# kmaninis/OSVOS-PyTorch

Hardware: NVIDIA H100
Metric: frames/sec at 480x854 fwd-only, batch 1 per GPU (OSVOS.forward -> 5 logit maps) (higher is better)
Workload: dtype bf16x3 (split-bf16 operands, fp32 accumulate)

## Files before the change

osvos_pytorch_b200/csrc/conv_stage1_fused.cu:

```cuda
#include <stdlib.h>
#include <string.h>

#include "conv_common.cuh"

namespace osvos {

constexpr int kS1Pitch = 10;
constexpr int kS1HaloRows = kTileH + 2;
constexpr int kS1HaloPx = kS1HaloRows * kS1Pitch;
constexpr int kS1APlane = (kS1HaloPx * 128 + 1023) / 1024 * 1024;
constexpr int kS1AStage = 2 * kS1APlane;
constexpr int kS1AStages = 2;
constexpr int kS1BPlane = 64 * 128;
constexpr int kS1BStage = 2 * kS1BPlane;
constexpr int kS1BStages = 5;
constexpr int kS1W1Bytes = (64 * 27 + 64) * 4;
constexpr int kS1Builders = 96;
constexpr int kS1Smem = kS1AStages * kS1AStage + kS1BStages * kS1BStage + kS1W1Bytes + 1024 + 512;
static_assert(kS1Smem <= 227 * 1024, "stage-1 kernel exceeds the per-CTA shared memory");
static_assert(kS1Smem + 4096 < (1 << 18), "descriptor start-address field would overflow");

struct Stage1Params {
  const float* x;
  const float* w1;
  const float* b1;
};

__global__ void __launch_bounds__(kConvThreads, 1)
conv_stage1_fused_kernel(const __grid_constant__ CUtensorMap map_w_hi, const __grid_constant__ CUtensorMap map_w_lo,
                         const Stage1Params s1, const ConvParams p) {
  extern __shared__ uint8_t smem_raw[];
  uint8_t* smem = reinterpret_cast<uint8_t*>((reinterpret_cast<uintptr_t>(smem_raw) + 1023) & ~uintptr_t(1023));
  uint8_t* smem_a = smem;
  uint8_t* smem_b = smem_a + kS1AStages * kS1AStage;
  float* w1s = reinterpret_cast<float*>(smem_b + kS1BStages * kS1BStage);
  uint64_t* bars = reinterpret_cast<uint64_t*>(reinterpret_cast<uint8_t*>(w1s) + kS1W1Bytes);
  uint64_t* a_full = bars;
  uint64_t* a_empty = bars + 2;
  uint64_t* b_full = bars + 4;
  uint64_t* b_empty = bars + 4 + kS1BStages;

  const int warp = threadIdx.x >> 5;
  const int lane = threadIdx.x & 31;

  if (threadIdx.x == 0) {
    tma_prefetch_desc(&map_w_hi);
    tma_prefetch_desc(&map_w_lo);
    for (int i = 0; i < 2; ++i) {
      mbar_init(&a_full[i], kS1Builders);
      mbar_init(&a_empty[i], 2);
    }
    for (int i = 0; i < kS1BStages; ++i) {
      mbar_init(&b_full[i], 1);
      mbar_init(&b_empty[i], 2);
    }
    fence_barrier_init();
  }
  pdl_wait();
  pdl_launch_dependents();
  for (int i = threadIdx.x; i < 64 * 27 + 64; i += kConvThreads)
    w1s[i] = i < 64 * 27 ? __ldg(s1.w1 + i) : (s1.b1 ? __ldg(s1.b1 + i - 64 * 27) : 0.f);
  __syncthreads();

  if (warp == 0) {
    if (elect_one()) {
      int b_stage = 0;
      uint32_t b_phase = 0;
      for (int tile = blockIdx.x; tile < p.total_tiles; tile += gridDim.x) {
#pragma unroll
        for (int tap = 0; tap < 9; ++tap) {
          mbar_wait(&b_empty[b_stage], b_phase ^ 1);
          uint8_t* st = smem_b + b_stage * kS1BStage;
          mbar_arrive_expect_tx(&b_full[b_stage], kS1BStage);
          tma_load_3d(&map_w_hi, &b_full[b_stage], st, 0, 0, tap);
          tma_load_3d(&map_w_lo, &b_full[b_stage], st + kS1BPlane, 0, 0, tap);
          if (++b_stage == kS1BStages) {
            b_stage = 0;
            b_phase ^= 1;
          }
        }
      }
    }
    __syncwarp();
  } else if (warp < 4) {
    const int t = threadIdx.x - 32;
    const size_t plane_sz = static_cast<size_t>(p.h) * p.w;
    int a_stage = 0;
    uint32_t a_phase = 0;
    for (int tile = blockIdx.x; tile < p.total_tiles; tile += gridDim.x) {
      int nb, tx, ty, img;
      decode_tile(p, tile, nb, tx, ty, img);
      mbar_wait(&a_empty[a_stage], a_phase ^ 1);
      uint8_t* st = smem_a + a_stage * kS1AStage;
      for (int pix = t; pix < kS1HaloPx; pix += kS1Builders) {
        const int hy = pix / kS1Pitch, hx = pix - hy * kS1Pitch;
        const int y = ty * kTileH - 1 + hy, xx = tx * kTileW - 1 + hx;
        const bool inside = y >= 0 && y < p.h && xx >= 0 && xx < p.w;
        float v[27];
#pragma unroll
        for (int ci = 0; ci < 3; ++ci) {
          const float* pl = s1.x + (static_cast<size_t>(img) * 3 + ci) * plane_sz;
#pragma unroll
          for (int r = 0; r < 3; ++r) {
            const int iy = y + r - 1;
#pragma unroll
            for (int s = 0; s < 3; ++s) {
              const int ix = xx + s - 1;
              v[ci * 9 + r * 3 + s] =
                  (inside && iy >= 0 && iy < p.h && ix >= 0 && ix < p.w) ? __ldg(pl + static_cast<size_t>(iy) * p.w + ix) : 0.f;
            }
          }
        }
#pragma unroll 1
        for (int chunk = 0; chunk < 8; ++chunk) {
          float f[8];
#pragma unroll
          for (int e = 0; e < 8; ++e) {
            const int co = chunk * 8 + e;
            float acc = w1s[64 * 27 + co];
#pragma unroll
            for (int k = 0; k < 27; ++k) acc = fmaf(w1s[co * 27 + k], v[k], acc);
            f[e] = inside ? fmaxf(acc, 0.f) : 0.f;
          }
          uint32_t hi[4], lo[4];
#pragma unroll
          for (int e = 0; e < 4; ++e) split_pack2(f[2 * e], f[2 * e + 1], hi[e], lo[e]);
          const uint32_t off = sw128_offset(pix, chunk);
          *reinterpret_cast<uint4*>(st + off) = make_uint4(hi[0], hi[1], hi[2], hi[3]);
          *reinterpret_cast<uint4*>(st + kS1APlane + off) = make_uint4(lo[0], lo[1], lo[2], lo[3]);
        }
      }
      fence_proxy_async_smem();
      mbar_arrive(&a_full[a_stage]);
      if (++a_stage == kS1AStages) {
        a_stage = 0;
        a_phase ^= 1;
      }
    }
  } else {
    const int wg = (warp - 4) >> 2, wl = warp & 3;
    const bool leader = (threadIdx.x & 127) == 0;
    constexpr uint64_t kDescA = desc_template(16, kS1Pitch * 128, kDescSW128);
    constexpr uint64_t kDescB = desc_template(16, 1024, kDescSW128);
    const uint32_t smem_a_u32 = smem_u32(smem_a) + wg * 8 * kS1Pitch * 128, smem_b_u32 = smem_u32(smem_b);
    float acc[64];
    int a_stage = 0, b_stage = 0;
    uint32_t a_phase = 0, b_phase = 0;
    StageRelease pending;
    for (int tile = blockIdx.x; tile < p.total_tiles; tile += gridDim.x) {
#pragma unroll
      for (int i = 0; i < 64; ++i) acc[i] = 0.f;
      mbar_wait(&a_full[a_stage], a_phase);
      const uint64_t da0 = kDescA | static_cast<uint64_t>((smem_a_u32 + a_stage * kS1AStage) >> 4);
#pragma unroll
      for (int tap = 0; tap < 9; ++tap) {
        const uint32_t tap_off = static_cast<uint32_t>(((tap / 3) * kS1Pitch + (tap % 3)) * (128 >> 4));
        mbar_wait(&b_full[b_stage], b_phase);
        const uint64_t db_hi = kDescB | static_cast<uint64_t>((smem_b_u32 + b_stage * kS1BStage) >> 4);
        const uint64_t da_hi = da0 + tap_off;
        const uint64_t da_lo = da_hi + (kS1APlane >> 4);
        wgmma_fence();
#pragma unroll
        for (int k = 0; k < kBlockK / 16; ++k) {
          wgmma_bf16<128>(acc, da_hi + 2 * k, db_hi + 2 * k, 1);
          wgmma_bf16<64>(acc, da_lo + 2 * k, db_hi + 2 * k, 1);
        }
        wgmma_commit();
        wgmma_wait<1>();
        pending.release(leader);
        pending.bar_b = &b_empty[b_stage];
        if (tap == 8) pending.bar_a = &a_empty[a_stage];
        if (++b_stage == kS1BStages) {
          b_stage = 0;
          b_phase ^= 1;
        }
      }
      if (++a_stage == kS1AStages) {
        a_stage = 0;
        a_phase ^= 1;
      }
      wgmma_wait<0>();
      wgmma_fence_operands(acc);
      pending.release(leader);
      conv_epilogue<64, true, true>(p, acc, tile, wg, wl, lane);
    }
  }
}

}

using namespace osvos;

extern "C" int osvos_stage1_fused(const osvos_stage1_args* a, osvos_stream_t stream_) {
  OSVOS_CHECK_ARG(a != nullptr && a->x != nullptr && a->w1 != nullptr && a->w2_packed != nullptr);
  OSVOS_CHECK_ARG(a->n > 0 && a->h > 0 && a->w > 0 && a->h <= 65535 && a->n <= 65535);
  OSVOS_CHECK_ARG((a->y_hi != nullptr && a->y_lo != nullptr) || (a->pool_hi != nullptr && a->pool_lo != nullptr));
  OSVOS_CHECK_ARG((a->y_hi == nullptr) == (a->y_lo == nullptr) && (a->pool_hi == nullptr) == (a->pool_lo == nullptr));
  {
    const uintptr_t any = reinterpret_cast<uintptr_t>(a->y_hi) | reinterpret_cast<uintptr_t>(a->y_lo) |
                          reinterpret_cast<uintptr_t>(a->pool_hi) | reinterpret_cast<uintptr_t>(a->pool_lo);
    OSVOS_CHECK_ARG((any & 3) == 0);
    OSVOS_CHECK_ARG(((reinterpret_cast<uintptr_t>(a->b1) | reinterpret_cast<uintptr_t>(a->b2) |
                      reinterpret_cast<uintptr_t>(a->w2_packed)) & 15) == 0);
  }
  cudaStream_t stream = static_cast<cudaStream_t>(stream_);
  osvos_conv3x3_args c;
  memset(&c, 0, sizeof(c));
  c.w_packed = a->w2_packed;
  c.bias = a->b2;
  c.y_hi = a->y_hi;
  c.y_lo = a->y_lo;
  c.pool_hi = a->pool_hi;
  c.pool_lo = a->pool_lo;
  c.n = a->n, c.h = a->h, c.w = a->w, c.cin = 64, c.cout = 64;
  c.flags = OSVOS_FLAG_RELU;
  ConvParams p;
  fill_conv_params(p, &c, 64);
  CUtensorMap mw_hi, mw_lo;
  int rc = encode_weight_maps(&mw_hi, &mw_lo, &c, 64);
  if (rc) return rc;
  Stage1Params s1;
  s1.x = a->x;
  s1.w1 = a->w1;
  s1.b1 = a->b1;
  const int sms = device_sm_count();
  const int grid = p.total_tiles < sms ? p.total_tiles : sms;
  auto kern = conv_stage1_fused_kernel;
  static uint64_t attr_done = 0;
  OSVOS_CHECK_CUDA(ensure_dynamic_smem(kern, kS1Smem, &attr_done));
  OSVOS_CHECK_CUDA(launch_pdl(kern, dim3(grid), dim3(kConvThreads), kS1Smem, stream, mw_hi, mw_lo, s1, p));
  return OSVOS_OK;
}
```

osvos_pytorch_b200/csrc/ptx.cuh:

```cuda
#pragma once
#include <cuda.h>
#include <cuda_runtime.h>
#include <stdint.h>

#include "wgmma.cuh"

namespace osvos {

#ifndef OSVOS_SPIN_LIMIT
#define OSVOS_SPIN_LIMIT (1u << 26)
#endif

__device__ __forceinline__ uint32_t smem_u32(const void* p) {
  return static_cast<uint32_t>(__cvta_generic_to_shared(p));
}

__device__ __forceinline__ bool elect_one() {
  uint32_t pred = 0;
  asm volatile(
      "{\n\t.reg .pred P;\n\t"
      "elect.sync _|P, 0xffffffff;\n\t"
      "selp.u32 %0, 1, 0, P;\n\t}\n"
      : "=r"(pred));
  return pred != 0;
}

__device__ __forceinline__ void pdl_wait() { asm volatile("griddepcontrol.wait;" ::: "memory"); }
__device__ __forceinline__ void pdl_launch_dependents() { asm volatile("griddepcontrol.launch_dependents;" ::: "memory"); }

__device__ __forceinline__ void mbar_init(uint64_t* bar, uint32_t count) {
  asm volatile("mbarrier.init.shared::cta.b64 [%0], %1;" ::"r"(smem_u32(bar)), "r"(count) : "memory");
}
__device__ __forceinline__ void fence_barrier_init() {
  asm volatile("fence.mbarrier_init.release.cluster;" ::: "memory");
}
__device__ __forceinline__ void fence_proxy_async_smem() {
  asm volatile("fence.proxy.async.shared::cta;" ::: "memory");
}
__device__ __forceinline__ void mbar_arrive_expect_tx(uint64_t* bar, uint32_t bytes) {
  asm volatile("mbarrier.arrive.expect_tx.shared::cta.b64 _, [%0], %1;" ::"r"(smem_u32(bar)), "r"(bytes)
               : "memory");
}
__device__ __forceinline__ void mbar_arrive(uint64_t* bar) {
  asm volatile("mbarrier.arrive.shared::cta.b64 _, [%0];" ::"r"(smem_u32(bar)) : "memory");
}
__device__ __forceinline__ bool mbar_try_wait(uint64_t* bar, uint32_t parity) {
  uint32_t ok;
  asm volatile(
      "{\n\t.reg .pred P;\n\t"
      "mbarrier.try_wait.parity.shared::cta.b64 P, [%1], %2;\n\t"
      "selp.u32 %0, 1, 0, P;\n\t}\n"
      : "=r"(ok)
      : "r"(smem_u32(bar)), "r"(parity)
      : "memory");
  return ok != 0;
}

__device__ __forceinline__ void mbar_wait(uint64_t* bar, uint32_t parity) {
  uint32_t spins = 0;
  while (!mbar_try_wait(bar, parity)) {
    if (++spins > OSVOS_SPIN_LIMIT) __trap();
  }
}

__device__ __forceinline__ void cp_async_8_zfill(void* dst, const void* src, uint32_t src_bytes) {
  asm volatile("cp.async.ca.shared.global [%0], [%1], 8, %2;" ::"r"(smem_u32(dst)), "l"(src), "r"(src_bytes) : "memory");
}
__device__ __forceinline__ void cp_async_mbar_arrive_noinc(uint64_t* bar) {
  asm volatile("cp.async.mbarrier.arrive.noinc.shared::cta.b64 [%0];" ::"r"(smem_u32(bar)) : "memory");
}

__device__ __forceinline__ void tma_prefetch_desc(const CUtensorMap* m) {
  asm volatile("prefetch.tensormap [%0];" ::"l"(reinterpret_cast<uint64_t>(m)) : "memory");
}
__device__ __forceinline__ void tma_load_4d(const CUtensorMap* m, uint64_t* bar, void* dst, int c0, int c1, int c2,
                                            int c3) {
  asm volatile(
      "cp.async.bulk.tensor.4d.shared::cluster.global.mbarrier::complete_tx::bytes"
      " [%0], [%1, {%3, %4, %5, %6}], [%2];"
      ::"r"(smem_u32(dst)), "l"(reinterpret_cast<uint64_t>(m)), "r"(smem_u32(bar)), "r"(c0), "r"(c1), "r"(c2),
      "r"(c3)
      : "memory");
}
__device__ __forceinline__ void tma_load_2d(const CUtensorMap* m, uint64_t* bar, void* dst, int c0, int c1) {
  asm volatile(
      "cp.async.bulk.tensor.2d.shared::cluster.global.mbarrier::complete_tx::bytes"
      " [%0], [%1, {%3, %4}], [%2];"
      ::"r"(smem_u32(dst)), "l"(reinterpret_cast<uint64_t>(m)), "r"(smem_u32(bar)), "r"(c0), "r"(c1)
      : "memory");
}
__device__ __forceinline__ void tma_load_3d(const CUtensorMap* m, uint64_t* bar, void* dst, int c0, int c1, int c2) {
  asm volatile(
      "cp.async.bulk.tensor.3d.shared::cluster.global.mbarrier::complete_tx::bytes"
      " [%0], [%1, {%3, %4, %5}], [%2];"
      ::"r"(smem_u32(dst)), "l"(reinterpret_cast<uint64_t>(m)), "r"(smem_u32(bar)), "r"(c0), "r"(c1), "r"(c2)
      : "memory");
}
__device__ __forceinline__ void st_shared_u32(uint32_t addr, uint32_t v) {
  asm volatile("st.shared.u32 [%0], %1;" ::"r"(addr), "r"(v) : "memory");
}
__device__ __forceinline__ void tma_store_4d(const CUtensorMap* m, const void* src, int c0, int c1, int c2, int c3) {
  asm volatile(
      "cp.async.bulk.tensor.4d.global.shared::cta.bulk_group [%0, {%2, %3, %4, %5}], [%1];"
      ::"l"(reinterpret_cast<uint64_t>(m)), "r"(smem_u32(src)), "r"(c0), "r"(c1), "r"(c2), "r"(c3)
      : "memory");
}
__device__ __forceinline__ void bulk_commit_group() { asm volatile("cp.async.bulk.commit_group;" ::: "memory"); }
template <int N>
__device__ __forceinline__ void bulk_wait_group_read() { asm volatile("cp.async.bulk.wait_group.read %0;" ::"n"(N) : "memory"); }
template <int N>
__device__ __forceinline__ void bulk_wait_group() { asm volatile("cp.async.bulk.wait_group %0;" ::"n"(N) : "memory"); }

constexpr uint64_t kDescSW128 = 1ull << 62;
__host__ __device__ constexpr uint64_t desc_template(uint32_t lbo_bytes, uint32_t sbo_bytes, uint64_t layout) {
  return (static_cast<uint64_t>((lbo_bytes >> 4) & 0x3FFF) << 16) | (static_cast<uint64_t>((sbo_bytes >> 4) & 0x3FFF) << 32) |
         layout;
}
__device__ __forceinline__ uint64_t make_smem_desc(const void* p, uint32_t lbo_bytes, uint32_t sbo_bytes, uint64_t layout) {
  return desc_template(lbo_bytes, sbo_bytes, layout) | static_cast<uint64_t>((smem_u32(p) >> 4) & 0x3FFF);
}

__device__ __forceinline__ void named_bar_sync(int id, int nthreads) {
  asm volatile("bar.sync %0, %1;" ::"r"(id), "r"(nthreads) : "memory");
}
__device__ __forceinline__ void named_bar_arrive(int id, int nthreads) {
  asm volatile("bar.arrive %0, %1;" ::"r"(id), "r"(nthreads) : "memory");
}

template <int N>
__device__ __forceinline__ void setmaxnreg_dec() { asm volatile("setmaxnreg.dec.sync.aligned.u32 %0;" ::"n"(N)); }
template <int N>
__device__ __forceinline__ void setmaxnreg_inc() { asm volatile("setmaxnreg.inc.sync.aligned.u32 %0;" ::"n"(N)); }

struct StageRelease {
  uint64_t* bar_b = nullptr;
  uint64_t* bar_a = nullptr;
  __device__ __forceinline__ void release(bool leader) {
    if (leader) {
      if (bar_b) mbar_arrive(bar_b);
      if (bar_a) mbar_arrive(bar_a);
    }
    bar_b = bar_a = nullptr;
  }
};

}
```

osvos_pytorch_b200/csrc/wgmma.cuh:

```cuda
#pragma once
#include <stdint.h>

namespace osvos {

template <int N, int TA = 0, int TB = 0>
__device__ __forceinline__ void wgmma_bf16(float* d, uint64_t desc_a, uint64_t desc_b, uint32_t scale_d);

#define OSVOS_WGMMA_16(TA, TB)                                                                               \
  template <>                                                                                                  \
  __device__ __forceinline__ void wgmma_bf16<16, TA, TB>(float* d, uint64_t desc_a, uint64_t desc_b, uint32_t scale_d) { \
    asm volatile(                                                                                              \
        "{\n.reg .pred p;\nsetp.ne.b32 p, %10, 0;\n"                                                              \
        "wgmma.mma_async.sync.aligned.m64n16k16.f32.bf16.bf16 {%0, %1, %2, %3, %4, %5, %6, %7}, %8, %9, p, 1, 1, " #TA ", " #TB ";\n}\n" \
        : "+f"(d[0]), "+f"(d[1]), "+f"(d[2]), "+f"(d[3]), "+f"(d[4]), "+f"(d[5]), "+f"(d[6]), "+f"(d[7])                                                                                               \
        : "l"(desc_a), "l"(desc_b), "r"(scale_d) : "memory");                                                           \
  }
OSVOS_WGMMA_16(0, 0)
OSVOS_WGMMA_16(1, 1)
#undef OSVOS_WGMMA_16

#define OSVOS_WGMMA_32(TA, TB)                                                                               \
  template <>                                                                                                  \
  __device__ __forceinline__ void wgmma_bf16<32, TA, TB>(float* d, uint64_t desc_a, uint64_t desc_b, uint32_t scale_d) { \
    asm volatile(                                                                                              \
        "{\n.reg .pred p;\nsetp.ne.b32 p, %18, 0;\n"                                                              \
        "wgmma.mma_async.sync.aligned.m64n32k16.f32.bf16.bf16 {%0, %1, %2, %3, %4, %5, %6, %7, %8, %9, %10, %11, %12, %13, %14, %15}, %16, %17, p, 1, 1, " #TA ", " #TB ";\n}\n" \
        : "+f"(d[0]), "+f"(d[1]), "+f"(d[2]), "+f"(d[3]), "+f"(d[4]), "+f"(d[5]), "+f"(d[6]), "+f"(d[7]), "+f"(d[8]), "+f"(d[9]), "+f"(d[10]), "+f"(d[11]), "+f"(d[12]), "+f"(d[13]), "+f"(d[14]), "+f"(d[15])                                                                                               \
        : "l"(desc_a), "l"(desc_b), "r"(scale_d) : "memory");                                                           \
  }
OSVOS_WGMMA_32(0, 0)
OSVOS_WGMMA_32(1, 1)
#undef OSVOS_WGMMA_32

#define OSVOS_WGMMA_64(TA, TB)                                                                               \
  template <>                                                                                                  \
  __device__ __forceinline__ void wgmma_bf16<64, TA, TB>(float* d, uint64_t desc_a, uint64_t desc_b, uint32_t scale_d) { \
    asm volatile(                                                                                              \
        "{\n.reg .pred p;\nsetp.ne.b32 p, %34, 0;\n"                                                              \
        "wgmma.mma_async.sync.aligned.m64n64k16.f32.bf16.bf16 {%0, %1, %2, %3, %4, %5, %6, %7, %8, %9, %10, %11, %12, %13, %14, %15, %16, %17, %18, %19, %20, %21, %22, %23, %24, %25, %26, %27, %28, %29, %30, %31}, %32, %33, p, 1, 1, " #TA ", " #TB ";\n}\n" \
        : "+f"(d[0]), "+f"(d[1]), "+f"(d[2]), "+f"(d[3]), "+f"(d[4]), "+f"(d[5]), "+f"(d[6]), "+f"(d[7]), "+f"(d[8]), "+f"(d[9]), "+f"(d[10]), "+f"(d[11]), "+f"(d[12]), "+f"(d[13]), "+f"(d[14]), "+f"(d[15]), "+f"(d[16]), "+f"(d[17]), "+f"(d[18]), "+f"(d[19]), "+f"(d[20]), "+f"(d[21]), "+f"(d[22]), "+f"(d[23]), "+f"(d[24]), "+f"(d[25]), "+f"(d[26]), "+f"(d[27]), "+f"(d[28]), "+f"(d[29]), "+f"(d[30]), "+f"(d[31])                                                                                               \
        : "l"(desc_a), "l"(desc_b), "r"(scale_d) : "memory");                                                           \
  }
OSVOS_WGMMA_64(0, 0)
OSVOS_WGMMA_64(1, 1)
#undef OSVOS_WGMMA_64

#define OSVOS_WGMMA_128(TA, TB)                                                                               \
  template <>                                                                                                  \
  __device__ __forceinline__ void wgmma_bf16<128, TA, TB>(float* d, uint64_t desc_a, uint64_t desc_b, uint32_t scale_d) { \
    asm volatile(                                                                                              \
        "{\n.reg .pred p;\nsetp.ne.b32 p, %66, 0;\n"                                                              \
        "wgmma.mma_async.sync.aligned.m64n128k16.f32.bf16.bf16 {%0, %1, %2, %3, %4, %5, %6, %7, %8, %9, %10, %11, %12, %13, %14, %15, %16, %17, %18, %19, %20, %21, %22, %23, %24, %25, %26, %27, %28, %29, %30, %31, %32, %33, %34, %35, %36, %37, %38, %39, %40, %41, %42, %43, %44, %45, %46, %47, %48, %49, %50, %51, %52, %53, %54, %55, %56, %57, %58, %59, %60, %61, %62, %63}, %64, %65, p, 1, 1, " #TA ", " #TB ";\n}\n" \
        : "+f"(d[0]), "+f"(d[1]), "+f"(d[2]), "+f"(d[3]), "+f"(d[4]), "+f"(d[5]), "+f"(d[6]), "+f"(d[7]), "+f"(d[8]), "+f"(d[9]), "+f"(d[10]), "+f"(d[11]), "+f"(d[12]), "+f"(d[13]), "+f"(d[14]), "+f"(d[15]), "+f"(d[16]), "+f"(d[17]), "+f"(d[18]), "+f"(d[19]), "+f"(d[20]), "+f"(d[21]), "+f"(d[22]), "+f"(d[23]), "+f"(d[24]), "+f"(d[25]), "+f"(d[26]), "+f"(d[27]), "+f"(d[28]), "+f"(d[29]), "+f"(d[30]), "+f"(d[31]), "+f"(d[32]), "+f"(d[33]), "+f"(d[34]), "+f"(d[35]), "+f"(d[36]), "+f"(d[37]), "+f"(d[38]), "+f"(d[39]), "+f"(d[40]), "+f"(d[41]), "+f"(d[42]), "+f"(d[43]), "+f"(d[44]), "+f"(d[45]), "+f"(d[46]), "+f"(d[47]), "+f"(d[48]), "+f"(d[49]), "+f"(d[50]), "+f"(d[51]), "+f"(d[52]), "+f"(d[53]), "+f"(d[54]), "+f"(d[55]), "+f"(d[56]), "+f"(d[57]), "+f"(d[58]), "+f"(d[59]), "+f"(d[60]), "+f"(d[61]), "+f"(d[62]), "+f"(d[63])                                                                                               \
        : "l"(desc_a), "l"(desc_b), "r"(scale_d) : "memory");                                                           \
  }
OSVOS_WGMMA_128(0, 0)
OSVOS_WGMMA_128(1, 1)
#undef OSVOS_WGMMA_128

#define OSVOS_WGMMA_144(TA, TB)                                                                               \
  template <>                                                                                                  \
  __device__ __forceinline__ void wgmma_bf16<144, TA, TB>(float* d, uint64_t desc_a, uint64_t desc_b, uint32_t scale_d) { \
    asm volatile(                                                                                              \
        "{\n.reg .pred p;\nsetp.ne.b32 p, %74, 0;\n"                                                              \
        "wgmma.mma_async.sync.aligned.m64n144k16.f32.bf16.bf16 {%0, %1, %2, %3, %4, %5, %6, %7, %8, %9, %10, %11, %12, %13, %14, %15, %16, %17, %18, %19, %20, %21, %22, %23, %24, %25, %26, %27, %28, %29, %30, %31, %32, %33, %34, %35, %36, %37, %38, %39, %40, %41, %42, %43, %44, %45, %46, %47, %48, %49, %50, %51, %52, %53, %54, %55, %56, %57, %58, %59, %60, %61, %62, %63, %64, %65, %66, %67, %68, %69, %70, %71}, %72, %73, p, 1, 1, " #TA ", " #TB ";\n}\n" \
        : "+f"(d[0]), "+f"(d[1]), "+f"(d[2]), "+f"(d[3]), "+f"(d[4]), "+f"(d[5]), "+f"(d[6]), "+f"(d[7]), "+f"(d[8]), "+f"(d[9]), "+f"(d[10]), "+f"(d[11]), "+f"(d[12]), "+f"(d[13]), "+f"(d[14]), "+f"(d[15]), "+f"(d[16]), "+f"(d[17]), "+f"(d[18]), "+f"(d[19]), "+f"(d[20]), "+f"(d[21]), "+f"(d[22]), "+f"(d[23]), "+f"(d[24]), "+f"(d[25]), "+f"(d[26]), "+f"(d[27]), "+f"(d[28]), "+f"(d[29]), "+f"(d[30]), "+f"(d[31]), "+f"(d[32]), "+f"(d[33]), "+f"(d[34]), "+f"(d[35]), "+f"(d[36]), "+f"(d[37]), "+f"(d[38]), "+f"(d[39]), "+f"(d[40]), "+f"(d[41]), "+f"(d[42]), "+f"(d[43]), "+f"(d[44]), "+f"(d[45]), "+f"(d[46]), "+f"(d[47]), "+f"(d[48]), "+f"(d[49]), "+f"(d[50]), "+f"(d[51]), "+f"(d[52]), "+f"(d[53]), "+f"(d[54]), "+f"(d[55]), "+f"(d[56]), "+f"(d[57]), "+f"(d[58]), "+f"(d[59]), "+f"(d[60]), "+f"(d[61]), "+f"(d[62]), "+f"(d[63]), "+f"(d[64]), "+f"(d[65]), "+f"(d[66]), "+f"(d[67]), "+f"(d[68]), "+f"(d[69]), "+f"(d[70]), "+f"(d[71])                                                                                               \
        : "l"(desc_a), "l"(desc_b), "r"(scale_d) : "memory");                                                           \
  }
OSVOS_WGMMA_144(0, 0)
OSVOS_WGMMA_144(1, 1)
#undef OSVOS_WGMMA_144

#define OSVOS_WGMMA_256(TA, TB)                                                                               \
  template <>                                                                                                  \
  __device__ __forceinline__ void wgmma_bf16<256, TA, TB>(float* d, uint64_t desc_a, uint64_t desc_b, uint32_t scale_d) { \
    asm volatile(                                                                                              \
        "{\n.reg .pred p;\nsetp.ne.b32 p, %130, 0;\n"                                                              \
        "wgmma.mma_async.sync.aligned.m64n256k16.f32.bf16.bf16 {%0, %1, %2, %3, %4, %5, %6, %7, %8, %9, %10, %11, %12, %13, %14, %15, %16, %17, %18, %19, %20, %21, %22, %23, %24, %25, %26, %27, %28, %29, %30, %31, %32, %33, %34, %35, %36, %37, %38, %39, %40, %41, %42, %43, %44, %45, %46, %47, %48, %49, %50, %51, %52, %53, %54, %55, %56, %57, %58, %59, %60, %61, %62, %63, %64, %65, %66, %67, %68, %69, %70, %71, %72, %73, %74, %75, %76, %77, %78, %79, %80, %81, %82, %83, %84, %85, %86, %87, %88, %89, %90, %91, %92, %93, %94, %95, %96, %97, %98, %99, %100, %101, %102, %103, %104, %105, %106, %107, %108, %109, %110, %111, %112, %113, %114, %115, %116, %117, %118, %119, %120, %121, %122, %123, %124, %125, %126, %127}, %128, %129, p, 1, 1, " #TA ", " #TB ";\n}\n" \
        : "+f"(d[0]), "+f"(d[1]), "+f"(d[2]), "+f"(d[3]), "+f"(d[4]), "+f"(d[5]), "+f"(d[6]), "+f"(d[7]), "+f"(d[8]), "+f"(d[9]), "+f"(d[10]), "+f"(d[11]), "+f"(d[12]), "+f"(d[13]), "+f"(d[14]), "+f"(d[15]), "+f"(d[16]), "+f"(d[17]), "+f"(d[18]), "+f"(d[19]), "+f"(d[20]), "+f"(d[21]), "+f"(d[22]), "+f"(d[23]), "+f"(d[24]), "+f"(d[25]), "+f"(d[26]), "+f"(d[27]), "+f"(d[28]), "+f"(d[29]), "+f"(d[30]), "+f"(d[31]), "+f"(d[32]), "+f"(d[33]), "+f"(d[34]), "+f"(d[35]), "+f"(d[36]), "+f"(d[37]), "+f"(d[38]), "+f"(d[39]), "+f"(d[40]), "+f"(d[41]), "+f"(d[42]), "+f"(d[43]), "+f"(d[44]), "+f"(d[45]), "+f"(d[46]), "+f"(d[47]), "+f"(d[48]), "+f"(d[49]), "+f"(d[50]), "+f"(d[51]), "+f"(d[52]), "+f"(d[53]), "+f"(d[54]), "+f"(d[55]), "+f"(d[56]), "+f"(d[57]), "+f"(d[58]), "+f"(d[59]), "+f"(d[60]), "+f"(d[61]), "+f"(d[62]), "+f"(d[63]), "+f"(d[64]), "+f"(d[65]), "+f"(d[66]), "+f"(d[67]), "+f"(d[68]), "+f"(d[69]), "+f"(d[70]), "+f"(d[71]), "+f"(d[72]), "+f"(d[73]), "+f"(d[74]), "+f"(d[75]), "+f"(d[76]), "+f"(d[77]), "+f"(d[78]), "+f"(d[79]), "+f"(d[80]), "+f"(d[81]), "+f"(d[82]), "+f"(d[83]), "+f"(d[84]), "+f"(d[85]), "+f"(d[86]), "+f"(d[87]), "+f"(d[88]), "+f"(d[89]), "+f"(d[90]), "+f"(d[91]), "+f"(d[92]), "+f"(d[93]), "+f"(d[94]), "+f"(d[95]), "+f"(d[96]), "+f"(d[97]), "+f"(d[98]), "+f"(d[99]), "+f"(d[100]), "+f"(d[101]), "+f"(d[102]), "+f"(d[103]), "+f"(d[104]), "+f"(d[105]), "+f"(d[106]), "+f"(d[107]), "+f"(d[108]), "+f"(d[109]), "+f"(d[110]), "+f"(d[111]), "+f"(d[112]), "+f"(d[113]), "+f"(d[114]), "+f"(d[115]), "+f"(d[116]), "+f"(d[117]), "+f"(d[118]), "+f"(d[119]), "+f"(d[120]), "+f"(d[121]), "+f"(d[122]), "+f"(d[123]), "+f"(d[124]), "+f"(d[125]), "+f"(d[126]), "+f"(d[127])                                                                                               \
        : "l"(desc_a), "l"(desc_b), "r"(scale_d) : "memory");                                                           \
  }
OSVOS_WGMMA_256(0, 0)
OSVOS_WGMMA_256(1, 1)
#undef OSVOS_WGMMA_256


__device__ __forceinline__ void wgmma_fence() { asm volatile("wgmma.fence.sync.aligned;" ::: "memory"); }
__device__ __forceinline__ void wgmma_commit() { asm volatile("wgmma.commit_group.sync.aligned;" ::: "memory"); }
template <int N>
__device__ __forceinline__ void wgmma_wait() { asm volatile("wgmma.wait_group.sync.aligned %0;" ::"n"(N) : "memory"); }
template <int N>
__device__ __forceinline__ void wgmma_fence_operands(float (&d)[N]) {
#pragma unroll
  for (int i = 0; i < N; ++i) asm volatile("" : "+f"(d[i])::"memory");
}

}
```

Baseline: 656.0.

## Compute stage-1 conv1 on tensor cores with per-warpgroup ping-pong tile building

The first 3->64 convolution, previously computed with scalar FMAs by three builder warps, now runs as register-sourced wgmma (im2col fragments from a cp.async-staged input patch, split-bf16 weights in shared memory). Each consumer warpgroup builds its own halo tile and then runs both M halves of the conv2 GEMM, alternating between the two warpgroups through named barriers so that one builds while the other issues MMAs. Register budgets are rebalanced with setmaxnreg, and the weight pipeline is deepened to 7 stages. Ablation flags are also added. The change adds scheduling complexity and removes A-stage double buffering across tiles within a warpgroup.

```diff
diff --git a/osvos_pytorch_b200/csrc/conv_stage1_fused.cu b/osvos_pytorch_b200/csrc/conv_stage1_fused.cu
--- a/osvos_pytorch_b200/csrc/conv_stage1_fused.cu
+++ b/osvos_pytorch_b200/csrc/conv_stage1_fused.cu
@@ -8,17 +8,19 @@
 constexpr int kS1Pitch = 10;
 constexpr int kS1HaloRows = kTileH + 2;
 constexpr int kS1HaloPx = kS1HaloRows * kS1Pitch;
+constexpr int kS1Blocks = (kS1HaloPx + 63) / 64;
 constexpr int kS1APlane = (kS1HaloPx * 128 + 1023) / 1024 * 1024;
 constexpr int kS1AStage = 2 * kS1APlane;
-constexpr int kS1AStages = 2;
 constexpr int kS1BPlane = 64 * 128;
 constexpr int kS1BStage = 2 * kS1BPlane;
-constexpr int kS1BStages = 5;
-constexpr int kS1W1Bytes = (64 * 27 + 64) * 4;
-constexpr int kS1Builders = 96;
-constexpr int kS1Smem = kS1AStages * kS1AStage + kS1BStages * kS1BStage + kS1W1Bytes + 1024 + 512;
+constexpr int kS1BStages = 7;
+constexpr int kS1W1Plane = 64 * 128;
+constexpr int kS1InH = kTileH + 4, kS1InW = kTileW + 4;
+constexpr int kS1InFloats = 3 * kS1InH * kS1InW;
+constexpr int kS1Smem = 2 * kS1AStage + kS1BStages * kS1BStage + 2 * kS1W1Plane + 2 * kS1InFloats * 4 + 1024 + 128;
 static_assert(kS1Smem <= 227 * 1024, "stage-1 kernel exceeds the per-CTA shared memory");
 static_assert(kS1Smem + 4096 < (1 << 18), "descriptor start-address field would overflow");
+static_assert(kS1Blocks == 3 && kS1APlane / 128 >= kS1HaloPx, "halo rows and the stage plane disagree");
 
 struct Stage1Params {
   const float* x;
@@ -26,19 +28,61 @@
   const float* b1;
 };
 
+struct S1Frag {
+  uint32_t hi[2][4], lo[2][4];
+};
+
+__device__ __forceinline__ S1Frag s1_load_frag(const float* in, int pix0, int lane) {
+  S1Frag f;
+  int off[8];
+  bool kv[8];
+#pragma unroll
+  for (int i = 0; i < 8; ++i) {
+    const int k = (i >> 2) * 16 + ((i >> 1) & 1) * 8 + 2 * (lane & 3) + (i & 1);
+    const int ci = k / 9, r = (k % 9) / 3, s = k % 3;
+    off[i] = (ci * kS1InH + r) * kS1InW + s;
+    kv[i] = k < 27;
+  }
+  int base[2];
+  bool real[2];
+#pragma unroll
+  for (int h = 0; h < 2; ++h) {
+    const int pix = pix0 + 8 * h;
+    const int hy = pix / kS1Pitch, hx = pix - hy * kS1Pitch;
+    base[h] = hy * kS1InW + hx;
+    real[h] = pix < kS1HaloPx;
+  }
+#pragma unroll
+  for (int ks = 0; ks < 2; ++ks)
+#pragma unroll
+    for (int q = 0; q < 4; ++q) {
+      const int h = q & 1, i = ks * 4 + (q >> 1) * 2;
+      const float v0 = kv[i] && real[h] ? in[base[h] + off[i]] : 0.f;
+      const float v1 = kv[i + 1] && real[h] ? in[base[h] + off[i + 1]] : 0.f;
+      __nv_bfloat16 h0, l0, h1, l1;
+      split_bf16(v0, h0, l0);
+      split_bf16(v1, h1, l1);
+      f.hi[ks][q] = pack_bf16x2(h0, h1);
+      f.lo[ks][q] = pack_bf16x2(l0, l1);
+    }
+  return f;
+}
+
 __global__ void __launch_bounds__(kConvThreads, 1)
 conv_stage1_fused_kernel(const __grid_constant__ CUtensorMap map_w_hi, const __grid_constant__ CUtensorMap map_w_lo,
                          const Stage1Params s1, const ConvParams p) {
+  constexpr int SB = kS1BStages;
   extern __shared__ uint8_t smem_raw[];
   uint8_t* smem = reinterpret_cast<uint8_t*>((reinterpret_cast<uintptr_t>(smem_raw) + 1023) & ~uintptr_t(1023));
   uint8_t* smem_a = smem;
-  uint8_t* smem_b = smem_a + kS1AStages * kS1AStage;
-  float* w1s = reinterpret_cast<float*>(smem_b + kS1BStages * kS1BStage);
-  uint64_t* bars = reinterpret_cast<uint64_t*>(reinterpret_cast<uint8_t*>(w1s) + kS1W1Bytes);
-  uint64_t* a_full = bars;
-  uint64_t* a_empty = bars + 2;
-  uint64_t* b_full = bars + 4;
-  uint64_t* b_empty = bars + 4 + kS1BStages;
+  uint8_t* smem_b = smem_a + 2 * kS1AStage;
+  uint8_t* smem_w1 = smem_b + SB * kS1BStage;
+  float* smem_in = reinterpret_cast<float*>(smem_w1 + 2 * kS1W1Plane);
+  uint64_t* bars = reinterpret_cast<uint64_t*>(smem_in + 2 * kS1InFloats);
+  uint64_t* b_full = bars;
+  uint64_t* b_empty = bars + SB;
+  uint64_t* in_full = bars + 2 * SB;
+  uint64_t* in_empty = bars + 2 * SB + 2;
 
   const int warp = threadIdx.x >> 5;
   const int lane = threadIdx.x & 31;
@@ -46,144 +90,230 @@
   if (threadIdx.x == 0) {
     tma_prefetch_desc(&map_w_hi);
     tma_prefetch_desc(&map_w_lo);
+    for (int i = 0; i < SB; ++i) {
+      mbar_init(&b_full[i], 1);
+      mbar_init(&b_empty[i], 1);
+    }
     for (int i = 0; i < 2; ++i) {
-      mbar_init(&a_full[i], kS1Builders);
-      mbar_init(&a_empty[i], 2);
-    }
-    for (int i = 0; i < kS1BStages; ++i) {
-      mbar_init(&b_full[i], 1);
-      mbar_init(&b_empty[i], 2);
+      mbar_init(&in_full[i], 32);
+      mbar_init(&in_empty[i], 128);
     }
     fence_barrier_init();
   }
   pdl_wait();
   pdl_launch_dependents();
-  for (int i = threadIdx.x; i < 64 * 27 + 64; i += kConvThreads)
-    w1s[i] = i < 64 * 27 ? __ldg(s1.w1 + i) : (s1.b1 ? __ldg(s1.b1 + i - 64 * 27) : 0.f);
+  for (int i = threadIdx.x; i < 64 * 4; i += kConvThreads) {
+    const int co = i >> 2, chunk = i & 3;
+    uint32_t hi[4], lo[4];
+#pragma unroll
+    for (int t = 0; t < 4; ++t) {
+      const int k0 = chunk * 8 + 2 * t;
+      const float v0 = k0 < 27 ? s1.w1[co * 27 + k0] : 0.f;
+      const float v1 = k0 + 1 < 27 ? s1.w1[co * 27 + k0 + 1] : 0.f;
+      __nv_bfloat16 h0, l0, h1, l1;
+      split_bf16(v0, h0, l0);
+      split_bf16(v1, h1, l1);
+      hi[t] = pack_bf16x2(h0, h1);
+      lo[t] = pack_bf16x2(l0, l1);
+    }
+    *reinterpret_cast<uint4*>(smem_w1 + sw128_offset(co, chunk)) = make_uint4(hi[0], hi[1], hi[2], hi[3]);
+    *reinterpret_cast<uint4*>(smem_w1 + kS1W1Plane + sw128_offset(co, chunk)) = make_uint4(lo[0], lo[1], lo[2], lo[3]);
+  }
+  fence_proxy_async_smem();
   __syncthreads();
 
-  if (warp == 0) {
-    if (elect_one()) {
-      int b_stage = 0;
-      uint32_t b_phase = 0;
-      for (int tile = blockIdx.x; tile < p.total_tiles; tile += gridDim.x) {
-#pragma unroll
-        for (int tap = 0; tap < 9; ++tap) {
-          mbar_wait(&b_empty[b_stage], b_phase ^ 1);
-          uint8_t* st = smem_b + b_stage * kS1BStage;
-          mbar_arrive_expect_tx(&b_full[b_stage], kS1BStage);
-          tma_load_3d(&map_w_hi, &b_full[b_stage], st, 0, 0, tap);
-          tma_load_3d(&map_w_lo, &b_full[b_stage], st + kS1BPlane, 0, 0, tap);
-          if (++b_stage == kS1BStages) {
-            b_stage = 0;
-            b_phase ^= 1;
-          }
-        }
-      }
-    }
-    __syncwarp();
-  } else if (warp < 4) {
-    const int t = threadIdx.x - 32;
-    const size_t plane_sz = static_cast<size_t>(p.h) * p.w;
-    int a_stage = 0;
-    uint32_t a_phase = 0;
-    for (int tile = blockIdx.x; tile < p.total_tiles; tile += gridDim.x) {
-      int nb, tx, ty, img;
-      decode_tile(p, tile, nb, tx, ty, img);
-      mbar_wait(&a_empty[a_stage], a_phase ^ 1);
-      uint8_t* st = smem_a + a_stage * kS1AStage;
-      for (int pix = t; pix < kS1HaloPx; pix += kS1Builders) {
-        const int hy = pix / kS1Pitch, hx = pix - hy * kS1Pitch;
-        const int y = ty * kTileH - 1 + hy, xx = tx * kTileW - 1 + hx;
-        const bool inside = y >= 0 && y < p.h && xx >= 0 && xx < p.w;
-        float v[27];
-#pragma unroll
-        for (int ci = 0; ci < 3; ++ci) {
-          const float* pl = s1.x + (static_cast<size_t>(img) * 3 + ci) * plane_sz;
-#pragma unroll
-          for (int r = 0; r < 3; ++r) {
-            const int iy = y + r - 1;
-#pragma unroll
-            for (int s = 0; s < 3; ++s) {
-              const int ix = xx + s - 1;
-              v[ci * 9 + r * 3 + s] =
-                  (inside && iy >= 0 && iy < p.h && ix >= 0 && ix < p.w) ? __ldg(pl + static_cast<size_t>(iy) * p.w + ix) : 0.f;
+  if (warp < 4) {
+    setmaxnreg_dec<40>();
+    if (warp == 0) {
+      if (elect_one()) {
+        const bool skip_b = (p.ablate & 1) != 0;
+        int b_stage = 0;
+        uint32_t b_phase = 0;
+        for (int tile = blockIdx.x; tile < p.total_tiles; tile += gridDim.x) {
+#pragma unroll
+          for (int tap = 0; tap < 9; ++tap) {
+            mbar_wait(&b_empty[b_stage], b_phase ^ 1);
+            if (skip_b) {
+              mbar_arrive(&b_full[b_stage]);
+            } else {
+              uint8_t* st = smem_b + b_stage * kS1BStage;
+              mbar_arrive_expect_tx(&b_full[b_stage], kS1BStage);
+              tma_load_3d(&map_w_hi, &b_full[b_stage], st, 0, 0, tap);
+              tma_load_3d(&map_w_lo, &b_full[b_stage], st + kS1BPlane, 0, 0, tap);
+            }
+            if (++b_stage == SB) {
+              b_stage = 0;
+              b_phase ^= 1;
             }
           }
         }
-#pragma unroll 1
-        for (int chunk = 0; chunk < 8; ++chunk) {
-          float f[8];
-#pragma unroll
-          for (int e = 0; e < 8; ++e) {
-            const int co = chunk * 8 + e;
-            float acc = w1s[64 * 27 + co];
-#pragma unroll
-            for (int k = 0; k < 27; ++k) acc = fmaf(w1s[co * 27 + k], v[k], acc);
-            f[e] = inside ? fmaxf(acc, 0.f) : 0.f;
-          }
-          uint32_t hi[4], lo[4];
-#pragma unroll
-          for (int e = 0; e < 4; ++e) split_pack2(f[2 * e], f[2 * e + 1], hi[e], lo[e]);
-          const uint32_t off = sw128_offset(pix, chunk);
-          *reinterpret_cast<uint4*>(st + off) = make_uint4(hi[0], hi[1], hi[2], hi[3]);
-          *reinterpret_cast<uint4*>(st + kS1APlane + off) = make_uint4(lo[0], lo[1], lo[2], lo[3]);
-        }
-      }
-      fence_proxy_async_smem();
-      mbar_arrive(&a_full[a_stage]);
-      if (++a_stage == kS1AStages) {
-        a_stage = 0;
-        a_phase ^= 1;
-      }
-    }
-  } else {
-    const int wg = (warp - 4) >> 2, wl = warp & 3;
-    const bool leader = (threadIdx.x & 127) == 0;
-    constexpr uint64_t kDescA = desc_template(16, kS1Pitch * 128, kDescSW128);
-    constexpr uint64_t kDescB = desc_template(16, 1024, kDescSW128);
-    const uint32_t smem_a_u32 = smem_u32(smem_a) + wg * 8 * kS1Pitch * 128, smem_b_u32 = smem_u32(smem_b);
-    float acc[64];
-    int a_stage = 0, b_stage = 0;
-    uint32_t a_phase = 0, b_phase = 0;
-    StageRelease pending;
-    for (int tile = blockIdx.x; tile < p.total_tiles; tile += gridDim.x) {
-#pragma unroll
-      for (int i = 0; i < 64; ++i) acc[i] = 0.f;
-      mbar_wait(&a_full[a_stage], a_phase);
-      const uint64_t da0 = kDescA | static_cast<uint64_t>((smem_a_u32 + a_stage * kS1AStage) >> 4);
-#pragma unroll
-      for (int tap = 0; tap < 9; ++tap) {
-        const uint32_t tap_off = static_cast<uint32_t>(((tap / 3) * kS1Pitch + (tap % 3)) * (128 >> 4));
-        mbar_wait(&b_full[b_stage], b_phase);
-        const uint64_t db_hi = kDescB | static_cast<uint64_t>((smem_b_u32 + b_stage * kS1BStage) >> 4);
-        const uint64_t da_hi = da0 + tap_off;
-        const uint64_t da_lo = da_hi + (kS1APlane >> 4);
-        wgmma_fence();
-#pragma unroll
-        for (int k = 0; k < kBlockK / 16; ++k) {
-          wgmma_bf16<128>(acc, da_hi + 2 * k, db_hi + 2 * k, 1);
-          wgmma_bf16<64>(acc, da_lo + 2 * k, db_hi + 2 * k, 1);
-        }
-        wgmma_commit();
-        wgmma_wait<1>();
-        pending.release(leader);
-        pending.bar_b = &b_empty[b_stage];
-        if (tap == 8) pending.bar_a = &a_empty[a_stage];
-        if (++b_stage == kS1BStages) {
-          b_stage = 0;
-          b_phase ^= 1;
-        }
-      }
-      if (++a_stage == kS1AStages) {
-        a_stage = 0;
-        a_phase ^= 1;
-      }
+      }
+      __syncwarp();
+    } else if (warp < 3) {
+      const int g = warp - 1;
+      float* in = smem_in + g * kS1InFloats;
+      const size_t plane_sz = static_cast<size_t>(p.h) * p.w;
+      const bool skip_in = (p.ablate & 2) != 0;
+      for (int k = g, use = 0;; k += 2, ++use) {
+        const int tile = static_cast<int>(blockIdx.x) + k * static_cast<int>(gridDim.x);
+        if (tile >= p.total_tiles) break;
+        int nb, tx, ty, img;
+        decode_tile(p, tile, nb, tx, ty, img);
+        const int y0 = ty * kTileH - 2, x0 = tx * kTileW - 2;
+        const float* src = s1.x + static_cast<size_t>(img) * 3 * plane_sz;
+        mbar_wait(&in_empty[g], (use & 1) ^ 1);
+        if (skip_in) {
+          mbar_arrive(&in_full[g]);
+          continue;
+        }
+        for (int i = lane; i < kS1InFloats; i += 32) {
+          const int ci = i / (kS1InH * kS1InW), rem = i - ci * (kS1InH * kS1InW);
+          const int yy = y0 + rem / kS1InW, xx = x0 + rem % kS1InW;
+          const bool inside = yy >= 0 && yy < p.h && xx >= 0 && xx < p.w;
+          cp_async_4_zfill(in + i, inside ? src + ci * plane_sz + static_cast<size_t>(yy) * p.w + xx : s1.x,
+                           inside ? 4 : 0);
+        }
+        cp_async_mbar_arrive_noinc(&in_full[g]);
+      }
+    }
+    return;
+  }
+
+  setmaxnreg_inc<232>();
+  const int wg = (warp - 4) >> 2, wl = warp & 3;
+  const int tid = threadIdx.x & 127;
+  const bool leader = tid == 0;
+  const int bar_build = 3 + wg;
+  constexpr uint64_t kDescA = desc_template(16, kS1Pitch * 128, kDescSW128);
+  constexpr uint64_t kDescB = desc_template(16, 1024, kDescSW128);
+  constexpr uint32_t kLoPlaneA = kS1APlane >> 4;
+  constexpr uint32_t kHalfA = (8 * kS1Pitch * 128) >> 4;
+  uint8_t* st_a = smem_a + wg * kS1AStage;
+  const uint32_t smem_b_u32 = smem_u32(smem_b);
+  const uint64_t da0 = kDescA | static_cast<uint64_t>(smem_u32(st_a) >> 4);
+  const float* in = smem_in + wg * kS1InFloats;
+  const bool skip_mma = (p.ablate & 4) != 0;
+
+  const uint64_t dw_hi = make_smem_desc(smem_w1, 16, 1024, kDescSW128), dw_lo = dw_hi + (kS1W1Plane >> 4);
+
+  auto issue = [&](float (&c)[32], const S1Frag& a) {
+#pragma unroll
+    for (int i = 0; i < 32; ++i) c[i] = 0.f;
+    wgmma_fence_operands(c);
+    wgmma_fence();
+    if (!skip_mma) {
+#pragma unroll
+      for (int k = 0; k < 2; ++k) {
+        wgmma_bf16_rs64(c, a.lo[k], dw_hi + 2 * k, 1);
+        wgmma_bf16_rs64(c, a.hi[k], dw_lo + 2 * k, 1);
+        wgmma_bf16_rs64(c, a.hi[k], dw_hi + 2 * k, 1);
+      }
+    }
+    wgmma_commit();
+  };
+  auto finish = [&](const float (&c)[32], int blk, int tx, int ty) {
+#pragma unroll
+    for (int h = 0; h < 2; ++h) {
+      const int pix = 64 * blk + 16 * wl + (lane >> 2) + 8 * h;
+      const int hy = pix / kS1Pitch, hx = pix - hy * kS1Pitch;
+      const int y = ty * kTileH - 1 + hy, x = tx * kTileW - 1 + hx;
+      const bool inside = pix < kS1HaloPx && y >= 0 && y < p.h && x >= 0 && x < p.w;
+      const uint32_t row_hi = smem_u32(st_a) + pix * 128 + 4 * (lane & 3);
+#pragma unroll
+      for (int j = 0; j < 8; ++j) {
+        const int ch = 8 * j + 2 * (lane & 3);
+        const float2 b = s1.b1 ? __ldg(reinterpret_cast<const float2*>(s1.b1 + ch)) : make_float2(0.f, 0.f);
+        float f[2];
+#pragma unroll
+        for (int e = 0; e < 2; ++e) {
+          float v = e ? b.y : b.x;
+          v += c[4 * j + 2 * h + e];
+          f[e] = inside ? fmaxf(v, 0.f) : 0.f;
+        }
+        if (pix < kS1HaloPx) {
+          uint32_t hi, lo;
+          split_pack2(f[0], f[1], hi, lo);
+          const uint32_t addr = row_hi + ((j ^ (pix & 7)) << 4);
+          st_shared_u32(addr, hi);
+          st_shared_u32(addr + kS1APlane, lo);
+        }
+      }
+    }
+  };
+  auto build = [&](int tile, int use) {
+    int nb, tx, ty, img;
+    decode_tile(p, tile, nb, tx, ty, img);
+    const int pix0 = 16 * wl + (lane >> 2);
+    float c[32];
+    named_bar_sync(bar_build, 128);
+    mbar_wait(&in_full[wg], use & 1);
+    if (p.ablate & 2) {
+      mbar_arrive(&in_empty[wg]);
+      return;
+    }
+#pragma unroll
+    for (int blk = 0; blk < kS1Blocks; ++blk) {
+      const S1Frag f = s1_load_frag(in, pix0 + 64 * blk, lane);
+      if (blk == kS1Blocks - 1) mbar_arrive(&in_empty[wg]);
+      issue(c, f);
       wgmma_wait<0>();
-      wgmma_fence_operands(acc);
+      wgmma_fence_operands(c);
+      finish(c, blk, tx, ty);
+    }
+    fence_proxy_async_smem();
+    named_bar_sync(bar_build, 128);
+  };
+
+  float acc[2][64];
+  StageRelease pending;
+  for (int k = wg;; k += 2) {
+    const int tile = static_cast<int>(blockIdx.x) + k * static_cast<int>(gridDim.x);
+    if (tile >= p.total_tiles) break;
+    const bool has_next = tile + static_cast<int>(gridDim.x) < p.total_tiles;
+    const int b_seq = 9 * k;
+    int b_stage = b_seq % SB;
+    uint32_t b_phase = (b_seq / SB) & 1;
+    build(tile, k >> 1);
+    if (k > 0) named_bar_sync(1 + wg, 256);
+#pragma unroll
+    for (int h = 0; h < 2; ++h)
+#pragma unroll
+      for (int i = 0; i < 64; ++i) acc[h][i] = 0.f;
+#pragma unroll
+    for (int h = 0; h < 2; ++h) wgmma_fence_operands(acc[h]);
+#pragma unroll
+    for (int tap = 0; tap < 9; ++tap) {
+      const uint32_t tap_off = static_cast<uint32_t>(((tap / 3) * kS1Pitch + (tap % 3)) * (128 >> 4));
+      mbar_wait(&b_full[b_stage], b_phase);
+      if (tap == 8 && has_next) named_bar_arrive(1 + (wg ^ 1), 256);
+      const uint64_t db_hi = kDescB | static_cast<uint64_t>((smem_b_u32 + b_stage * kS1BStage) >> 4);
+      wgmma_fence();
+#pragma unroll
+      for (int h = 0; h < 2; ++h) {
+        const uint64_t da_hi = da0 + h * kHalfA + tap_off;
+        const uint64_t da_lo = da_hi + kLoPlaneA;
+        if (skip_mma) continue;
+#pragma unroll
+        for (int ks = 0; ks < kBlockK / 16; ++ks) {
+          wgmma_bf16<128>(acc[h], da_hi + 2 * ks, db_hi + 2 * ks, 1);
+          wgmma_bf16<64>(acc[h], da_lo + 2 * ks, db_hi + 2 * ks, 1);
+        }
+      }
+      wgmma_commit();
+      wgmma_wait<1>();
       pending.release(leader);
-      conv_epilogue<64, true, true>(p, acc, tile, wg, wl, lane);
-    }
+      pending.bar_b = &b_empty[b_stage];
+      if (++b_stage == SB) {
+        b_stage = 0;
+        b_phase ^= 1;
+      }
+    }
+    wgmma_wait<0>();
+#pragma unroll
+    for (int h = 0; h < 2; ++h) wgmma_fence_operands(acc[h]);
+    pending.release(leader);
+#pragma unroll
+    for (int h = 0; h < 2; ++h) conv_epilogue<64, true, true>(p, acc[h], tile, h, wl, lane);
   }
 }
 
diff --git a/osvos_pytorch_b200/csrc/ptx.cuh b/osvos_pytorch_b200/csrc/ptx.cuh
--- a/osvos_pytorch_b200/csrc/ptx.cuh
+++ b/osvos_pytorch_b200/csrc/ptx.cuh
@@ -65,6 +65,9 @@
 
 __device__ __forceinline__ void cp_async_8_zfill(void* dst, const void* src, uint32_t src_bytes) {
   asm volatile("cp.async.ca.shared.global [%0], [%1], 8, %2;" ::"r"(smem_u32(dst)), "l"(src), "r"(src_bytes) : "memory");
+}
+__device__ __forceinline__ void cp_async_4_zfill(void* dst, const void* src, uint32_t src_bytes) {
+  asm volatile("cp.async.ca.shared.global [%0], [%1], 4, %2;" ::"r"(smem_u32(dst)), "l"(src), "r"(src_bytes) : "memory");
 }
 __device__ __forceinline__ void cp_async_mbar_arrive_noinc(uint64_t* bar) {
   asm volatile("cp.async.mbarrier.arrive.noinc.shared::cta.b64 [%0];" ::"r"(smem_u32(bar)) : "memory");
diff --git a/osvos_pytorch_b200/csrc/wgmma.cuh b/osvos_pytorch_b200/csrc/wgmma.cuh
--- a/osvos_pytorch_b200/csrc/wgmma.cuh
+++ b/osvos_pytorch_b200/csrc/wgmma.cuh
@@ -84,6 +84,13 @@
 OSVOS_WGMMA_256(1, 1)
 #undef OSVOS_WGMMA_256
 
+__device__ __forceinline__ void wgmma_bf16_rs64(float* d, const uint32_t (&a)[4], uint64_t desc_b, uint32_t scale_d) {
+  asm volatile(
+      "{\n.reg .pred p;\nsetp.ne.b32 p, %37, 0;\n"
+      "wgmma.mma_async.sync.aligned.m64n64k16.f32.bf16.bf16 {%0, %1, %2, %3, %4, %5, %6, %7, %8, %9, %10, %11, %12, %13, %14, %15, %16, %17, %18, %19, %20, %21, %22, %23, %24, %25, %26, %27, %28, %29, %30, %31}, {%32, %33, %34, %35}, %36, p, 1, 1, 0;\n}\n"
+      : "+f"(d[0]), "+f"(d[1]), "+f"(d[2]), "+f"(d[3]), "+f"(d[4]), "+f"(d[5]), "+f"(d[6]), "+f"(d[7]), "+f"(d[8]), "+f"(d[9]), "+f"(d[10]), "+f"(d[11]), "+f"(d[12]), "+f"(d[13]), "+f"(d[14]), "+f"(d[15]), "+f"(d[16]), "+f"(d[17]), "+f"(d[18]), "+f"(d[19]), "+f"(d[20]), "+f"(d[21]), "+f"(d[22]), "+f"(d[23]), "+f"(d[24]), "+f"(d[25]), "+f"(d[26]), "+f"(d[27]), "+f"(d[28]), "+f"(d[29]), "+f"(d[30]), "+f"(d[31])
+      : "r"(a[0]), "r"(a[1]), "r"(a[2]), "r"(a[3]), "l"(desc_b), "r"(scale_d) : "memory");
+}
 
 __device__ __forceinline__ void wgmma_fence() { asm volatile("wgmma.fence.sync.aligned;" ::: "memory"); }
 __device__ __forceinline__ void wgmma_commit() { asm volatile("wgmma.commit_group.sync.aligned;" ::: "memory"); }
```

After: 657.1 (median of 6 runs). About the same (+0.2%).
